# nobkagit/NeuralSteganography

Hardware: AMD Instinct MI355X
Metric: payload bits/sec + cover tokens/sec, GPT-2 arithmetic stego at batch, 1-8 GPUs (higher is better)
Workload: dtype f64; 1 GPU; C3 lockstep steps: gpt2 (random-init weights, fp16 compute, f16 logits, fp16 KV cache, batch-invariant native decode step) + ns_encode_step (temp 0.9, precision 26, topk 300), 4096 streams/GPU from a 32-token context, 262 timed lockstep steps (captured hipGraph replays) after 5 untimed, in 1 pass(es) of at most 1024 steps; global_batch=4096, vocab=50257, precision=26, topk=300, parallelism=dp1 (independent streams, no collective), model=gpt2 (random-init), lm_dtype=fp16, logits_dtype=f16, payload_bytes=1024

## Files before the change

### neuralsteganography_amd/csrc/nsg_coder.hip

```cpp

#include <hip/hip_runtime.h>
#include <stdint.h>
#include <stdio.h>
#include <stdlib.h>
#include <string.h>

#include <algorithm>
#include <string>

#include "../../include/nsg_coder.h"

#pragma clang fp contract(off)

#include "nsg_common.h"
#include "nsg_host.h"
#include "nsg_host.h"

#ifndef NSG_SAMPLE
#define NSG_SAMPLE 64
#endif
#ifndef NSG_FMA_ARG
#define NSG_FMA_ARG 1
#endif
#ifndef NSG_ASM_APPEND
// ... 1443 lines not shown
        s.bit_pos = 0;
        s.ntokens = 0;
        s.flags = 0;
        st[b] = s;
    }
}

}


static thread_local std::string g_err;

static int fail(ns_ctx* ctx, int code, const std::string& msg) {
    if (ctx)
        ctx->err = msg;
    else
        g_err = msg;
    return code;
}

static int g_split_max_b = -2;

static int split_setting() {
    if (g_split_max_b == -2) {
        const char* e = getenv("NSG_SPLIT_MAX_B");
        g_split_max_b = e ? std::max(0, atoi(e)) : -1;
    }
    return g_split_max_b;
}

static int split_max_b(int nsplit) {
    const int v = split_setting();
    return v >= 0 ? v : 6144 / nsplit;
}

template <typename T, bool DECODE, int NSK>
static void launch_one(const nsg::StepParams& p, hipStream_t s) {
    constexpr int NSPLIT = (64 * NSG_SAMPLE) / (nsg::WAVE * nsg::Elem<T>::W);
    if (p.spec_j > 0 && p.B <= split_max_b(NSPLIT)) {
        if (!DECODE && p.stats)
            hipLaunchKernelGGL((nsg::coder_step_kernel<T, DECODE, NSK, !DECODE, NSPLIT>), dim3(p.B),
                               dim3(NSPLIT * nsg::WAVE), 0, s, p);
        else
            hipLaunchKernelGGL((nsg::coder_step_kernel<T, DECODE, NSK, false, NSPLIT>), dim3(p.B),
                               dim3(NSPLIT * nsg::WAVE), 0, s, p);
        return;
    }
    const dim3 grid((p.B + nsg::WPB - 1) / nsg::WPB), block(nsg::WPB * nsg::WAVE);
    if (!DECODE && p.stats)
        hipLaunchKernelGGL((nsg::coder_step_kernel<T, DECODE, NSK, !DECODE>), grid, block, 0, s, p);
    else
        hipLaunchKernelGGL((nsg::coder_step_kernel<T, DECODE, NSK, false>), grid, block, 0, s, p);
}

template <typename T, bool DECODE>
static void launch_t(const nsg::StepParams& p, hipStream_t s) {
    if (p.K <= 128)
        launch_one<T, DECODE, 2>(p, s);
    else if (p.K <= 320)
        launch_one<T, DECODE, 5>(p, s);
    else if (p.K <= 512)
        launch_one<T, DECODE, 8>(p, s);
    else
        launch_one<T, DECODE, (nsg::CAND - nsg::WAVE * 4) / nsg::WAVE>(p, s);
}

template <bool DECODE>
static bool launch(ns_ctx* ctx, const nsg::StepParams& p, hipStream_t s) {
    if (ctx->dtype == NS_DTYPE_F16) {
        if (p.K <= 128)
            launch_one<_Float16, DECODE, 2>(p, s);
        else if (p.K <= 320)
            launch_one<_Float16, DECODE, 5>(p, s);
        else
            launch_one<_Float16, DECODE, (nsg::CAND - nsg::WAVE * 8) / nsg::WAVE>(p, s);
    } else {
        launch_t<float, DECODE>(p, s);
    }
    return hipGetLastError() == hipSuccess;
}

extern "C" {

const char* ns_version(void) { return "nsgcoder 0.25 gfx950"; }

int ns_set_split_max_batch(int max_batch) {
    const int prev = split_setting();
    g_split_max_b = max_batch < 0 ? -1 : max_batch;
    return prev;
}

int ns_max_topk(int logits_dtype) {
    if (logits_dtype == NS_DTYPE_F64) return 0;
    const int TS = (logits_dtype == NS_DTYPE_F16) ? nsg::WAVE * 8 : nsg::WAVE * 4;
    return nsg::CAND - TS;
}

const char* ns_last_error(const ns_ctx* ctx) { return ctx ? ctx->err.c_str() : g_err.c_str(); }

ns_ctx* ns_create(int device, int max_batch, int vocab, int max_k, int precision, int logits_dtype) {
    if (max_batch < 1 || vocab < 2 || max_k < 1 || precision < 1 || precision > 60 ||
        (logits_dtype != NS_DTYPE_F32 && logits_dtype != NS_DTYPE_F16 && logits_dtype != NS_DTYPE_F64)) {
        fail(nullptr, NS_ERR_CONFIG, "ns_create: invalid argument");
        return nullptr;
    }
    if (max_k > ns_max_topk(logits_dtype) && vocab > 0x1FFFF) {
        fail(nullptr, NS_ERR_UNSUPPORTED, "ns_create: the wide (large top-k) path supports vocab < 131072");
        return nullptr;
    }
    if (hipSetDevice(device) != hipSuccess) {
        fail(nullptr, NS_ERR_HIP, "ns_create: hipSetDevice failed");
        return nullptr;
    }
    ns_ctx* ctx = new ns_ctx();
    ctx->device = device;
    ctx->max_batch = max_batch;
    ctx->vocab = vocab;
    ctx->max_k = max_k;
    ctx->precision = precision;
    ctx->dtype = logits_dtype;
    ctx->d_counters = nullptr;
    ctx->wide = NsgWide();
    ctx->sent_end = nullptr;
    ctx->stats = nullptr;
    ctx->ranked = nullptr;
    ctx->ranked_stride = 0;
    ctx->stamps = nullptr;
    ctx->rk_count = nullptr;
    ctx->rk_idmap = nullptr;
    ctx->rk_idmap_stride = 0;
    ctx->rk_dict = 0;
    const size_t cbytes = 4 * NS_COUNTER_SHARDS * sizeof(unsigned long long);
    if (hipMalloc((void**)&ctx->d_counters, cbytes) != hipSuccess || hipMemset(ctx->d_counters, 0, cbytes) != hipSuccess) {
        fail(nullptr, NS_ERR_HIP, "ns_create: hipMalloc failed");
        delete ctx;
        return nullptr;
    }
    if (max_k > ns_max_topk(logits_dtype) && nsg_wide_alloc(ctx) != NS_OK) {
        fail(nullptr, NS_ERR_HIP, "ns_create: allocation of the wide-path scratch failed");
        nsg_wide_free(ctx);
        (void)hipFree(ctx->d_counters);
        delete ctx;
        return nullptr;
    }
    return ctx;
}

void ns_destroy(ns_ctx* ctx) {
    if (!ctx) return;
    if (ctx->d_counters) (void)hipFree(ctx->d_counters);
    nsg_wide_free(ctx);
    delete ctx;
}

int ns_init_state(ns_ctx* ctx, ns_stream_state* d_state, int B, void* hip_stream) {
    if (!ctx || !d_state || B < 1 || B > ctx->max_batch) return fail(ctx, NS_ERR_CONFIG, "ns_init_state: bad argument");
    const int threads = 256;
    hipLaunchKernelGGL(nsg::init_state_kernel, dim3((B + threads - 1) / threads), dim3(threads), 0,
                       (hipStream_t)hip_stream, d_state, B, ctx->precision);
    if (hipGetLastError() != hipSuccess) return fail(ctx, NS_ERR_HIP, "ns_init_state: launch failed");
    return NS_OK;
}

static int prepare(ns_ctx* ctx, nsg::StepParams& p, const void* d_logits, int64_t ld, int B, double temp,
                   int topk, const int32_t* banned, int nbanned, ns_step_trace* d_trace, uint32_t flags,
                   ns_stream_state* d_state) {
    if (!ctx) return fail(ctx, NS_ERR_CONFIG, "null context");
// ... 290 lines not shown
```

### neuralsteganography_amd/csrc/nsg_lm.hip

```cpp

#include <hip/hip_runtime.h>
#include <stdint.h>

#include "nsg_coder.h"
#include "nsg_lm.h"

namespace nsg {
namespace lm {

typedef _Float16 f16;
typedef _Float16 f16x8 __attribute__((ext_vector_type(8)));
typedef _Float16 f16x4 __attribute__((ext_vector_type(4)));
typedef float f32x4 __attribute__((ext_vector_type(4)));

constexpr int BK = 64;

__device__ __forceinline__ f32x4 mfma16(f16x8 a, f16x8 b, f32x4 c) {
    return __builtin_amdgcn_mfma_f32_16x16x32_f16(a, b, c, 0, 0, 0);
}

__device__ __forceinline__ float gelu_tanh(float x) {
    const float u = 0.7978845608028654f * (x + 0.044715f * (x * x * x));
    const float e = __builtin_amdgcn_exp2f(u * -2.8853900817779268f);
    return x * __builtin_amdgcn_rcpf(1.0f + e);
}

__device__ __forceinline__ f16 to_f16(float v) {
    asm volatile("" : "+v"(v));
    return (f16)v;
}

template <int EPI>
__device__ __forceinline__ void store4(void* Y, int64_t ldy, const f16* __restrict__ bias, int m, int n, f32x4 acc) {
    float v[4];
    if (bias) {
        const f16x4 bb = *(const f16x4*)(bias + n);
#pragma unroll
        for (int r = 0; r < 4; ++r) v[r] = acc[r] + (float)bb[r];
    } else {
#pragma unroll
        for (int r = 0; r < 4; ++r) v[r] = acc[r];
    }
    if constexpr (EPI == NS_LM_EPI_STORE_F32) {
        float* y = (float*)Y + (int64_t)m * ldy + n;
        *(f32x4*)y = f32x4{v[0], v[1], v[2], v[3]};
    } else {
        f16* y = (f16*)Y + (int64_t)m * ldy + n;
        f16x4 o;
        if constexpr (EPI == NS_LM_EPI_RESIDUAL) {
            const f16x4 h = *(const f16x4*)y;
#pragma unroll
            for (int r = 0; r < 4; ++r) o[r] = to_f16((float)h[r] + v[r]);
        } else if constexpr (EPI == NS_LM_EPI_GELU) {
#pragma unroll
            for (int r = 0; r < 4; ++r) o[r] = to_f16(gelu_tanh(v[r]));
        } else {
#pragma unroll
            for (int r = 0; r < 4; ++r) o[r] = to_f16(v[r]);
        }
        *(f16x4*)y = o;
    }
}

template <int EPI>
__device__ __forceinline__ void store4_pre(void* Y, int64_t ldy, bool has_bias, f16x4 bb, f16x4 h, int m, int n,
                                           f32x4 acc) {
    float v[4];
#pragma unroll
    for (int r = 0; r < 4; ++r) v[r] = has_bias ? acc[r] + (float)bb[r] : acc[r];
    if constexpr (EPI == NS_LM_EPI_STORE_F32) {
        float* y = (float*)Y + (int64_t)m * ldy + n;
        *(f32x4*)y = f32x4{v[0], v[1], v[2], v[3]};
    } else {
        f16* y = (f16*)Y + (int64_t)m * ldy + n;
        f16x4 o;
        if constexpr (EPI == NS_LM_EPI_RESIDUAL) {
#pragma unroll
            for (int r = 0; r < 4; ++r) o[r] = to_f16((float)h[r] + v[r]);
        } else if constexpr (EPI == NS_LM_EPI_GELU) {
#pragma unroll
            for (int r = 0; r < 4; ++r) o[r] = to_f16(gelu_tanh(v[r]));
        } else {
#pragma unroll
            for (int r = 0; r < 4; ++r) o[r] = to_f16(v[r]);
        }
        *(f16x4*)y = o;
    }
}

__host__ __device__ constexpr int k_chains(int K) { return K <= 1024 ? 1 : K <= 2048 ? 2 : 4; }

template <int FM, int SK, int EPI, int NW = 4>
__global__ __launch_bounds__(64 * NW) void gemm_direct(const f16* __restrict__ X, int64_t ldx,
                                                       const f16* __restrict__ Wt, int64_t ldw,
                                                       const f16* __restrict__ bias, void* Y, int64_t ldy, int M, int N,
                                                       int K) {
    static_assert(NW % SK == 0, "a workgroup holds whole weight blocks");
    __shared__ f32x4 s_part[SK > 1 ? NW : 1][SK > 1 ? FM : 1][64];
    const int lane = threadIdx.x & 63, wave = threadIdx.x >> 6;
    const int nb = blockIdx.x * (NW / SK) + wave / SK;
    const int chain = wave % SK;
    const bool live = nb * 16 < N;
    const int m0 = blockIdx.y * 16 * FM;
    const int r = lane & 15, c = lane >> 4;
    const int KT = K / 64, TPC = (KT + SK - 1) / SK;
    const int k_begin = min(chain * TPC, KT) * 64, k_end = min((chain + 1) * TPC, KT) * 64;
    const f16* wrow = Wt + (int64_t)min(nb * 16 + r, N - 1) * ldw + c * 8;
    const f16* xrow[FM];
#pragma unroll
    for (int f = 0; f < FM; ++f) xrow[f] = X + (int64_t)min(m0 + f * 16 + r, M - 1) * ldx + c * 8;
    f32x4 acc[FM];
#pragma unroll
    for (int f = 0; f < FM; ++f) acc[f] = f32x4{0.f, 0.f, 0.f, 0.f};
    const int n = nb * 16 + 4 * c;
    const bool ep = live && n < N && (SK == 1 || chain == 0);
    f16x4 pb = {}, ph[FM];
#pragma unroll
    for (int f = 0; f < FM; ++f) ph[f] = f16x4{};
    if (ep) {
        if (bias) pb = *(const f16x4*)(bias + n);
        if constexpr (EPI == NS_LM_EPI_RESIDUAL) {
#pragma unroll
            for (int f = 0; f < FM; ++f) {
                const int m = m0 + f * 16 + r;
                if (m < M) ph[f] = *(const f16x4*)((const f16*)Y + (int64_t)m * ldy + n);
            }
        }
    }
    constexpr int U = FM == 1 ? 24 : FM == 2 ? 12 : 8;
    int k = k_begin;
    if (live) {
        for (; k + 32 * U <= k_end; k += 32 * U) {
            f16x8 a[U], b[U][FM];
#pragma unroll
            for (int u = 0; u < U; ++u) {
                a[u] = *(const f16x8*)(wrow + k + 32 * u);
#pragma unroll
                for (int f = 0; f < FM; ++f) b[u][f] = *(const f16x8*)(xrow[f] + k + 32 * u);
            }
            __builtin_amdgcn_sched_barrier(0);
#pragma unroll
            for (int u = 0; u < U; ++u)
#pragma unroll
                for (int f = 0; f < FM; ++f) acc[f] = mfma16(a[u], b[u][f], acc[f]);
        }
        for (; k < k_end; k += 32) {
            const f16x8 a = *(const f16x8*)(wrow + k);
#pragma unroll
            for (int f = 0; f < FM; ++f) acc[f] = mfma16(a, *(const f16x8*)(xrow[f] + k), acc[f]);
        }
    }
    if constexpr (SK > 1) {
#pragma unroll
        for (int f = 0; f < FM; ++f) s_part[wave][f][lane] = acc[f];
        __syncthreads();
        if (chain != 0) return;
        for (int q = 1; q < SK; ++q)
#pragma unroll
            for (int f = 0; f < FM; ++f) acc[f] += s_part[wave + q][f][lane];
    }
    if (!ep) return;
#pragma unroll
    for (int f = 0; f < FM; ++f) {
        const int m = m0 + f * 16 + r;
        if (m < M) store4_pre<EPI>(Y, ldy, bias != nullptr, pb, ph[f], m, n, acc[f]);
    }
}

__device__ __forceinline__ int swz(int row) { return (row >> 1) & 7; }
// ... 67 lines not shown
#pragma unroll
    for (int i = 0; i < FN; ++i)
#pragma unroll
        for (int j = 0; j < FM; ++j) acc[i][j] = f32x4{0.f, 0.f, 0.f, 0.f};

    const int KT = K / BK;
    const int SK = k_chains(K), TPC = (KT + SK - 1) / SK;
    const int fr = lane & 15, fc = lane >> 4;
#pragma unroll
    for (int s0 = 0; s0 < NST - 1; ++s0)
        if (s0 < KT) stage(s0, s0);
    int buf = 0;
    for (int kt = 0; kt < KT; ++kt) {
        const int ahead = KT - 1 - kt;
        if constexpr (NST >= 3) {
            if (ahead >= NST - 2) {
                wait_vm<GL * (NST - 2)>();
            } else if (NST >= 4 && ahead == 1) {
                wait_vm<GL>();
            } else {
                wait_vm<0>();
            }
            __builtin_amdgcn_s_barrier();
            asm volatile("" ::: "memory");
            if (ahead >= NST - 1) {
                int nb = buf + NST - 1;
                nb -= nb >= NST ? NST : 0;
                stage(kt + NST - 1, nb);
            }
        } else {
            if (ahead >= 1) {
                stage(kt + 1, buf ^ 1);
                wait_vm<GL>();
            } else {
                wait_vm<0>();
            }
            __builtin_amdgcn_s_barrier();
            asm volatile("" ::: "memory");
        }
        if constexpr (SPLIT) {
            if (kt > 0 && kt % TPC == 0) {
#pragma unroll
                for (int i = 0; i < FN; ++i)
#pragma unroll
                    for (int j = 0; j < FM; ++j) {
                        tot[i][j] = kt == TPC ? acc[i][j] : tot[i][j] + acc[i][j];
                        acc[i][j] = f32x4{0.f, 0.f, 0.f, 0.f};
                    }
            }
        }
        const char* base = smem + buf * ROWS * 128;
        f16x8 a[2][FN], b[2][FM];
#pragma unroll
        for (int kk = 0; kk < 2; ++kk) {
            const int ch = kk * 4 + fc;
#pragma unroll
            for (int i = 0; i < FN; ++i) {
                const int row = wn * FN * 16 + i * 16 + fr;
                a[kk][i] = *(const f16x8*)(base + row * 128 + ((ch ^ swz(row)) << 4));
            }
#pragma unroll
            for (int j = 0; j < FM; ++j) {
                const int row = BN + wm * FM * 16 + j * 16 + fr;
                b[kk][j] = *(const f16x8*)(base + row * 128 + ((ch ^ swz(row)) << 4));
            }
        }
#pragma unroll
        for (int kk = 0; kk < 2; ++kk)
#pragma unroll
            for (int i = 0; i < FN; ++i)
#pragma unroll
                for (int j = 0; j < FM; ++j) acc[i][j] = mfma16(a[kk][i], b[kk][j], acc[i][j]);
        if constexpr (NST == 2) lds_fence_barrier();
        buf = buf + 1 == NST ? 0 : buf + 1;
    }
    if constexpr (SPLIT) {
        if (KT > TPC) {
#pragma unroll
            for (int i = 0; i < FN; ++i)
#pragma unroll
                for (int j = 0; j < FM; ++j) acc[i][j] = tot[i][j] + acc[i][j];
        }
    }
#pragma unroll
    for (int i = 0; i < FN; ++i) {
        const int n = n0 + wn * FN * 16 + i * 16 + 4 * fc;
        if (n >= N) continue;
#pragma unroll
        for (int j = 0; j < FM; ++j) {
            const int m = m0 + wm * FM * 16 + j * 16 + fr;
            if (m < M) store4<EPI>(Y, ldy, bias, m, n, acc[i][j]);
        }
    }
}

constexpr int PB_BIAS_MAX = 4096;

template <int N_>
__device__ __forceinline__ void wait_vm_le(int n) {
    if constexpr (N_ > 0) {
        if (n >= N_) {
            wait_vm<N_>();
            return;
        }
        wait_vm_le<N_ - 8>(n);
    } else {
        wait_vm<0>();
    }
}

template <int NST, bool SPLIT, int EPI>
__global__ __launch_bounds__(256) void gemm_persist(const f16* __restrict__ X, int64_t ldx,
                                                    const f16* __restrict__ Wt, int64_t ldw,
                                                    const f16* __restrict__ bias, void* Y, int64_t ldy, int M, int N,
                                                    int K) {
    constexpr int BN = 128, BM = 128, WM = 2, NT = 256, NW = 4, FN = 4, FM = 4;
    constexpr int ROWS = BN + BM, GL = ROWS * 8 / NT, SB = ROWS * 128;
    constexpr int NSTO = FN * FM;
    constexpr int ESZ = EPI == NS_LM_EPI_STORE_F32 ? 4 : 2;
    static_assert(NST >= 2 && NST <= 4 && GL == 8, "ring");
    __shared__ __attribute__((aligned(16))) char smem[NST * SB + PB_BIAS_MAX * 2];
    f16* s_bias = (f16*)(smem + NST * SB);

    const int lane = threadIdx.x & 63, wave = threadIdx.x >> 6;
    const int wn = wave / WM, wm = wave - wn * WM;
    const int fr = lane & 15, fc = lane >> 4;
    const int tiles_m = (M + BM - 1) / BM, tiles_n = N / BN, T = tiles_m * tiles_n;
    const int G = gridDim.x, g = xcd_remap(blockIdx.x, G);
    const int KT = K / BK, SK = k_chains(K), TPC = (KT + SK - 1) / SK;
    const int ntl = g < T ? (T - 1 - g) / G + 1 : 0;
    const int S = ntl * KT;

    if (bias) {
        for (int i = threadIdx.x * 8; i < N; i += NT * 8) *(f16x8*)(s_bias + i) = *(const f16x8*)(bias + i);
    }
    __syncthreads();

    auto origin = [&](int i, int& n0, int& m0) {
        constexpr int GN = 1024 / BN;
        const int t = g + i * G;
        const int grp = t / (GN * tiles_m), within = t - grp * (GN * tiles_m);
        const int gn = min(GN, tiles_n - grp * GN);
        const int tm = within / gn;
        n0 = (grp * GN + (within - tm * gn)) * BN;
        m0 = tm * BM;
    };
    const int srow = lane >> 3;
    auto stage = [&](int i, int kt, int buf) {
        int n0, m0;
        origin(i, n0, m0);
        char* dst = smem + buf * SB;
#pragma unroll
        for (int q = 0; q < GL; ++q) {
            const int qq = q * NW + wave;
            const int row = qq * 8 + srow;
            const int chunk = (lane & 7) ^ swz(row);
            const f16* src = q < GL / 2 ? Wt + (int64_t)(n0 + row) * ldw
                                        : X + (int64_t)min(m0 + row - BN, M - 1) * ldx;
            __builtin_amdgcn_global_load_lds((const __attribute__((address_space(1))) void*)(src + chunk * 8 + kt * BK),
                                             (__attribute__((address_space(3))) void*)(dst + qq * 8 * 128), 16, 0, 0);
        }
    };

    const auto rs = __builtin_amdgcn_make_buffer_rsrc(Y, (short)0, (int)((int64_t)M * ldy * ESZ), 0x00020000);

    f32x4 acc[FN][FM];
    f32x4 tot[SPLIT ? FN : 1][SPLIT ? FM : 1];
#pragma unroll
    for (int i = 0; i < FN; ++i)
#pragma unroll
        for (int j = 0; j < FM; ++j) acc[i][j] = f32x4{0.f, 0.f, 0.f, 0.f};

    int is_i = 0, is_k = 0, is_n = 0;
    auto issue = [&]() {
        stage(is_i, is_k, is_n % NST);
        ++is_n;
// ... 230 lines not shown
        char* dst = smem + buf * SB;
        int r8 = wn * 8 + lr;
        asm volatile("" : "+v"(r8));
        if (g == 0) {
#pragma unroll
            for (int q = 0; q < WP + 4; ++q) {
                const f16* p = q < WP ? Wt + (int64_t)min(n0 + q * 32 + r8, N - 1) * ldw
                                      : X + (int64_t)min(m0 + (q - WP) * 32 + r8, M - 1) * ldx;
                __builtin_amdgcn_global_load_lds((const __attribute__((address_space(1))) void*)(p + chunk * 8 + kt * BK),
                                                 (__attribute__((address_space(3))) void*)(dst + (q * 4 + wn) * 1024),
                                                 16, 0, 0);
            }
        } else {
#pragma unroll
            for (int q = 0; q < 4; ++q) {
                const f16* p = X + (int64_t)min(m0 + 128 + q * 32 + r8, M - 1) * ldx;
                __builtin_amdgcn_global_load_lds((const __attribute__((address_space(1))) void*)(p + chunk * 8 + kt * BK),
                                                 (__attribute__((address_space(3))) void*)(dst + ((BN + 128) / 8 + q * 4 + wn) * 1024),
                                                 16, 0, 0);
            }
        }
    };
    auto barrier = []() {
        __builtin_amdgcn_sched_barrier(0);
        __builtin_amdgcn_s_barrier();
        asm volatile("" ::: "memory");
        __builtin_amdgcn_sched_barrier(0);
    };

    f32x4 acc[FN][FM];
#pragma unroll
    for (int i = 0; i < FN; ++i)
#pragma unroll
        for (int j = 0; j < FM; ++j) acc[i][j] = f32x4{0.f, 0.f, 0.f, 0.f};

    const int KT = K / BK;
    stage(0, 0);
    wait_vm<0>();
    barrier();
    if (g == 1) barrier();
    for (int kt = 0; kt < KT; ++kt) {
        const int buf = kt & 1;
        const char* base = smem + buf * SB;
        f16x8 a[2][FN], b[2][FM];
#pragma unroll
        for (int kk = 0; kk < 2; ++kk) {
            const int ch = kk * 4 + fc;
#pragma unroll
            for (int i = 0; i < FN; ++i) {
                const int row = wn * FN * 16 + i * 16 + fr;
                a[kk][i] = *(const f16x8*)(base + row * 128 + ((ch ^ swz(row)) << 4));
            }
#pragma unroll
            for (int j = 0; j < FM; ++j) {
                const int row = BN + g * FM * 16 + j * 16 + fr;
                b[kk][j] = *(const f16x8*)(base + row * 128 + ((ch ^ swz(row)) << 4));
            }
        }
        if (kt + 1 < KT) stage(kt + 1, buf ^ 1);
        asm volatile("s_waitcnt lgkmcnt(0)" ::: "memory");
        barrier();
        __builtin_amdgcn_s_setprio(1);
#pragma unroll
        for (int kk = 0; kk < 2; ++kk)
#pragma unroll
            for (int i = 0; i < FN; ++i)
#pragma unroll
                for (int j = 0; j < FM; ++j) acc[i][j] = mfma16(a[kk][i], b[kk][j], acc[i][j]);
        __builtin_amdgcn_s_setprio(0);
        if (kt + 1 < KT) wait_vm<0>();
        barrier();
    }
    if (g == 0) barrier();
#pragma unroll
    for (int i = 0; i < FN; ++i) {
        const int n = n0 + wn * FN * 16 + i * 16 + 4 * fc;
        if (n >= N) continue;
#pragma unroll
        for (int j = 0; j < FM; ++j) {
            const int m = m0 + g * FM * 16 + j * 16 + fr;
            if (m < M) store4<EPI>(Y, ldy, bias, m, n, acc[i][j]);
        }
    }
}

template <int SK, int EPI>
__global__ __launch_bounds__(256 * SK) void gemm_chains(const f16* __restrict__ X, int64_t ldx,
                                                         const f16* __restrict__ Wt, int64_t ldw,
                                                         const f16* __restrict__ bias, void* Y, int64_t ldy, int M,
                                                         int N, int K) {
    constexpr int BN = 64, BM = 64, WM = 2, FN = 2, FM = 2;
    constexpr int ROWS = BN + BM, GL = ROWS * 8 / 256;
    constexpr int SB = ROWS * 128;
    static_assert(SK == 2 || SK == 4, "chains");
    __shared__ __attribute__((aligned(16))) char smem[SK * 2 * SB];

    const int tiles_m = (M + BM - 1) / BM;
    const int tiles_n = (N + BN - 1) / BN;
    const int t = xcd_remap(blockIdx.x, tiles_m * tiles_n);
    constexpr int GN = 1024 / BN;
    const int grp = t / (GN * tiles_m), within = t - grp * (GN * tiles_m);
    const int gn = min(GN, tiles_n - grp * GN);
    const int tm = within / gn, tn = grp * GN + (within - tm * gn);
    const int n0 = tn * BN, m0 = tm * BM;
    const int lane = threadIdx.x & 63;
    const int wave = __builtin_amdgcn_readfirstlane(threadIdx.x >> 6);
    const int c = wave >> 2, ww = wave & 3;
    const int wn = ww / WM, wm = ww - wn * WM;
    char* ring = smem + c * 2 * SB;

    const f16* src[GL];
    int lds_off[GL];
#pragma unroll
    for (int g = 0; g < GL; ++g) {
        const int q = g * 4 + ww;
        const int row = q * 8 + (lane >> 3);
        const int chunk = (lane & 7) ^ swz(row);
        if (row < BN)
            src[g] = Wt + (int64_t)min(n0 + row, N - 1) * ldw + chunk * 8;
        else
            src[g] = X + (int64_t)min(m0 + row - BN, M - 1) * ldx + chunk * 8;
        lds_off[g] = q * 8 * 128;
    }
    auto stage = [&](int kt, int buf) {
#pragma unroll
        for (int g = 0; g < GL; ++g)
            __builtin_amdgcn_global_load_lds((const __attribute__((address_space(1))) void*)(src[g] + kt * BK),
                                             (__attribute__((address_space(3))) void*)(ring + buf * SB + lds_off[g]),
                                             16, 0, 0);
    };

    f32x4 acc[FN][FM];
#pragma unroll
    for (int i = 0; i < FN; ++i)
#pragma unroll
        for (int j = 0; j < FM; ++j) acc[i][j] = f32x4{0.f, 0.f, 0.f, 0.f};
    const int KT = K / BK, TPC = (KT + SK - 1) / SK;
    const int k0 = c * TPC, nk = max(0, min(k0 + TPC, KT) - k0);
    const int fr = lane & 15, fc = lane >> 4;
    if (nk > 0) stage(k0, 0);
    int buf = 0;
    for (int i = 0; i < TPC; ++i) {
        if (i + 1 < nk) {
            stage(k0 + i + 1, buf ^ 1);
            wait_vm<GL>();
        } else {
            wait_vm<0>();
        }
        __builtin_amdgcn_s_barrier();
        asm volatile("" ::: "memory");
        if (i < nk) {
            const char* base = ring + buf * SB;
            f16x8 a[2][FN], b[2][FM];
#pragma unroll
            for (int kk = 0; kk < 2; ++kk) {
                const int ch = kk * 4 + fc;
#pragma unroll
                for (int ii = 0; ii < FN; ++ii) {
                    const int row = wn * FN * 16 + ii * 16 + fr;
                    a[kk][ii] = *(const f16x8*)(base + row * 128 + ((ch ^ swz(row)) << 4));
                }
#pragma unroll
                for (int j = 0; j < FM; ++j) {
                    const int row = BN + wm * FM * 16 + j * 16 + fr;
                    b[kk][j] = *(const f16x8*)(base + row * 128 + ((ch ^ swz(row)) << 4));
                }
// ... 152 lines not shown
            for (int e = 0; e < 4; ++e) {
                h[e] = ok ? (f16)((float)te[e] + (float)tp[e]) : (f16)__builtin_nanf("");
                x[v][e] = (float)h[e];
            }
            *(f16x4*)(hr + 4 * i) = h;
        }
    }
    ln_row(x, NV4, C, w, b, A + (int64_t)row * lda, eps);
}


constexpr int LNG_MAXK = 1024;
template <int EPI, int NW = 4>
__global__ __launch_bounds__(64 * NW) void gemm_direct_ln(const f16* __restrict__ X, int64_t ldx,
                                                          const f16* __restrict__ lw, const f16* __restrict__ lb,
                                                          float eps, const f16* __restrict__ Wt, int64_t ldw,
                                                          const f16* __restrict__ bias, void* Y, int64_t ldy, int M,
                                                          int N, int K) {
    __shared__ __attribute__((aligned(16))) f16 sA[16][LNG_MAXK + 8];
    const int lane = threadIdx.x & 63, wave = threadIdx.x >> 6;
    const int nb = blockIdx.x * NW + wave;
    const bool live = nb * 16 < N;
    const int r = lane & 15, c = lane >> 4;
    const int KS = K / 32;
    const f16* wrow = Wt + (int64_t)min(nb * 16 + r, N - 1) * ldw + c * 8;
    f16x8 a[LNG_MAXK / 32];
    if (live) {
#pragma unroll
        for (int u = 0; u < LNG_MAXK / 32; ++u)
            if (u < KS) a[u] = *(const f16x8*)(wrow + 32 * u);
    }
    const int n = nb * 16 + 4 * c;
    const bool ep = live && n < N;
    f16x4 pb = {}, ph = {};
    if (ep) {
        if (bias) pb = *(const f16x4*)(bias + n);
        if constexpr (EPI == NS_LM_EPI_RESIDUAL) {
            if (r < M) ph = *(const f16x4*)((const f16*)Y + (int64_t)r * ldy + n);
        }
    }
    const int NV4 = K >> 2;
    for (int row = wave; row < M; row += NW) {
        const f16* xr = X + (int64_t)row * ldx;
        float x[LN_MAXV][4];
#pragma unroll
        for (int v = 0; v < LN_MAXV; ++v) {
            const int i = lane + 64 * v;
            if (i < NV4) {
                const f16x4 t = *(const f16x4*)(xr + 4 * i);
#pragma unroll
                for (int e = 0; e < 4; ++e) x[v][e] = (float)t[e];
            }
        }
        ln_row(x, NV4, K, lw, lb, &sA[row][0], eps);
    }
    __syncthreads();
    if (!ep) return;
    const f16* arow = &sA[min(r, M - 1)][c * 8];
    f32x4 acc = f32x4{0.f, 0.f, 0.f, 0.f};
#pragma unroll
    for (int u = 0; u < LNG_MAXK / 32; ++u)
        if (u < KS) acc = mfma16(a[u], *(const f16x8*)(arow + 32 * u), acc);
    if (r < M) store4_pre<EPI>(Y, ldy, bias != nullptr, pb, ph, r, n, acc);
}

}
}

using namespace nsg::lm;

enum GemmCfg {
    CFG_DIRECT16 = 0, CFG_DIRECT32, CFG_DIRECT64,
    CFG_T64_2, CFG_T64_3,
    CFG_T128_2, CFG_T128_3, CFG_T128_4,
    CFG_T256x128_2, CFG_T256x128_3,
    CFG_T128x256_2,
    CFG_T64_4,
    CFG_T128x64_3,
    CFG_B256,
    CFG_P128_2, CFG_P128_3, CFG_P128_4,
    CFG_PP256,
    CFG_PP192,
    CFG_C64,
    CFG_COUNT
};

static int cu_count() {
    static int n = 0;
    if (n == 0) {
        int dev = 0, v = 0;
        if (hipGetDevice(&dev) == hipSuccess &&
            hipDeviceGetAttribute(&v, hipDeviceAttributeMultiprocessorCount, dev) == hipSuccess && v > 0)
            n = v;
        else
            n = 256;
    }
    return n;
}

static bool persist_ok(int epi, const void* bias, int64_t ldy, int M, int N) {
    const int64_t esz = epi == NS_LM_EPI_STORE_F32 ? 4 : 2;
    return epi != NS_LM_EPI_RESIDUAL && N % 128 == 0 && (!bias || N <= PB_BIAS_MAX) &&
           ((int64_t)M + 128) * ldy * esz < ((int64_t)1 << 31);
}

#ifndef NSG_DIRECT_NW
#define NSG_DIRECT_NW 1
#endif

template <int FM, int EPI>
static void launch_direct(const f16* x, int64_t ldx, const f16* wt, int64_t ldw, const f16* bias, void* y,
                          int64_t ldy, int M, int N, int K, hipStream_t st) {
    const int nbk = N / 16, my = (M + 16 * FM - 1) / (16 * FM);
    constexpr int NW1 = NSG_DIRECT_NW;
    switch (k_chains(K)) {
        case 1:
            hipLaunchKernelGGL((gemm_direct<FM, 1, EPI, NW1>), dim3((nbk + NW1 - 1) / NW1, my), dim3(64 * NW1), 0, st,
                               x, ldx, wt, ldw, bias, y, ldy, M, N, K);
            break;
        case 2:
            hipLaunchKernelGGL((gemm_direct<FM, 2, EPI>), dim3((nbk + 1) / 2, my), dim3(256), 0, st, x, ldx, wt, ldw,
                               bias, y, ldy, M, N, K);
            break;
        default:
            hipLaunchKernelGGL((gemm_direct<FM, 4, EPI>), dim3(nbk, my), dim3(256), 0, st, x, ldx, wt, ldw, bias, y,
                               ldy, M, N, K);
            break;
    }
}

template <int EPI>
static void launch_cfg(int cfg, const f16* x, int64_t ldx, const f16* wt, int64_t ldw, const f16* bias, void* y,
                       int64_t ldy, int M, int N, int K, hipStream_t st) {
    auto tiles = [&](int bn, int bm) { return dim3((unsigned)(((M + bm - 1) / bm) * (long)((N + bn - 1) / bn))); };
    const bool split = k_chains(K) > 1;
    switch (cfg) {
#define NSG_DIRECT(FMv) launch_direct<FMv, EPI>(x, ldx, wt, ldw, bias, y, ldy, M, N, K, st)
#define NSG_TILED(BNv, BMv, WNv, WMv, NSTv)                                                                     \
    if (split)                                                                                                  \
        hipLaunchKernelGGL((gemm_tiled<BNv, BMv, WNv, WMv, NSTv, true, EPI>), tiles(BNv, BMv), dim3(64 * WNv * WMv), \
                           0, st, x, ldx, wt, ldw, bias, y, ldy, M, N, K);                                      \
    else                                                                                                        \
        hipLaunchKernelGGL((gemm_tiled<BNv, BMv, WNv, WMv, NSTv, false, EPI>), tiles(BNv, BMv),                 \
                           dim3(64 * WNv * WMv), 0, st, x, ldx, wt, ldw, bias, y, ldy, M, N, K)
        case CFG_DIRECT16: NSG_DIRECT(1); break;
        case CFG_DIRECT32: NSG_DIRECT(2); break;
        case CFG_DIRECT64: NSG_DIRECT(4); break;
        case CFG_T64_2: NSG_TILED(64, 64, 2, 2, 2); break;
        case CFG_T64_3: NSG_TILED(64, 64, 2, 2, 3); break;
        case CFG_T128_2: NSG_TILED(128, 128, 2, 2, 2); break;
        case CFG_T128_3: NSG_TILED(128, 128, 2, 2, 3); break;
        case CFG_T128_4: NSG_TILED(128, 128, 2, 2, 4); break;
        case CFG_T256x128_2: NSG_TILED(256, 128, 4, 2, 2); break;
        case CFG_T256x128_3: NSG_TILED(256, 128, 4, 2, 3); break;
        case CFG_T128x256_2: NSG_TILED(128, 256, 2, 4, 2); break;
        case CFG_T64_4: NSG_TILED(64, 64, 2, 2, 4); break;
        case CFG_T128x64_3: NSG_TILED(128, 64, 2, 2, 3); break;
        case CFG_B256:
            if (split) {
                NSG_TILED(128, 128, 2, 2, 2);
            } else {
                hipLaunchKernelGGL((gemm_big<EPI>), tiles(256, 256), dim3(512), 0, st, x, ldx, wt, ldw, bias, y, ldy,
                                   M, N, K);
            }
            break;
        case CFG_PP256:
            if (split) {
                NSG_TILED(128, 128, 2, 2, 2);
            } else {
                hipLaunchKernelGGL((gemm_pp<EPI>), tiles(256, 256), dim3(512), 0, st, x, ldx, wt, ldw, bias, y, ldy, M,
                                   N, K);
            }
            break;
        case CFG_PP192:
            if (split) {
                NSG_TILED(128, 128, 2, 2, 2);
            } else {
                hipLaunchKernelGGL((gemm_pp<EPI, 192>), tiles(192, 256), dim3(512), 0, st, x, ldx, wt, ldw, bias, y,
                                   ldy, M, N, K);
            }
            break;
        case CFG_C64: {
            const int sk = k_chains(K);
            if (sk == 4)
                hipLaunchKernelGGL((gemm_chains<4, EPI>), tiles(64, 64), dim3(1024), 0, st, x, ldx, wt, ldw, bias, y, ldy,
                                   M, N, K);
            else if (sk == 2)
                hipLaunchKernelGGL((gemm_chains<2, EPI>), tiles(64, 64), dim3(512), 0, st, x, ldx, wt, ldw, bias, y, ldy,
                                   M, N, K);
            else
                NSG_TILED(64, 64, 2, 2, 2);
            break;
        }
        case CFG_P128_2:
        case CFG_P128_3:
        case CFG_P128_4: {
            if (!persist_ok(EPI, bias, ldy, M, N)) {
                NSG_TILED(128, 128, 2, 2, 2);
                break;
            }
            const int T = ((M + 127) / 128) * (N / 128);
            const int G = min(T, cu_count() * (cfg == CFG_P128_2 ? 2 : 1));
            if constexpr (EPI != NS_LM_EPI_RESIDUAL) {
#define NSG_PERSIST(NSTv)                                                                                        \
    if (split)                                                                                                   \
        hipLaunchKernelGGL((gemm_persist<NSTv, true, EPI>), dim3(G), dim3(256), 0, st, x, ldx, wt, ldw, bias, y, \
                           ldy, M, N, K);                                                                        \
    else                                                                                                         \
        hipLaunchKernelGGL((gemm_persist<NSTv, false, EPI>), dim3(G), dim3(256), 0, st, x, ldx, wt, ldw, bias, y, \
                           ldy, M, N, K)
                if (cfg == CFG_P128_2) {
                    NSG_PERSIST(2);
                } else if (cfg == CFG_P128_3) {
                    NSG_PERSIST(3);
                } else {
                    NSG_PERSIST(4);
                }
#undef NSG_PERSIST
            }
            break;
        }
#undef NSG_DIRECT
#undef NSG_TILED
        default: break;
    }
}

static int auto_cfg(int M, int N, int K) {
    const bool split = k_chains(K) > 1;
    if (M <= 16) return (N >= 8192 && !split) ? CFG_T64_2 : CFG_DIRECT16;
    if (split && M <= 256) return M <= 64 ? CFG_DIRECT16 : M <= 128 ? CFG_DIRECT32 : CFG_DIRECT64;
    if (N >= 8192 && M >= 512) return (!split && M < 2048) ? CFG_PP256 : CFG_T128_2;
    if (!split && M >= 4096 && N >= 2048) {
        const long cu = cu_count(), tm = (M + 255) / 256;
        const long w256 = (tm * ((N + 255) / 256) + cu - 1) / cu * 256;
        const long w192 = (tm * ((N + 191) / 192) + cu - 1) / cu * 192;
        return w192 < w256 ? CFG_PP192 : CFG_PP256;
    }
    if (!split && M >= 1024 && N >= 4096) return CFG_T128x64_3;
    if (split && (long)((M + 63) / 64) * ((N + 63) / 64) <= 2L * cu_count()) return CFG_C64;
    return CFG_T64_2;
}

static int gemm_checked(const void* d_x, int64_t ldx, const void* d_wt, int64_t ldw, const void* d_bias, void* d_y,
                        int64_t ldy, int M, int N, int K, int epilogue, int cfg, void* hip_stream) {
    if (!d_x || !d_wt || !d_y || M <= 0 || N <= 0 || K <= 0) return NS_ERR_CONFIG;
    if (K % 64 || N % 16) return NS_ERR_UNSUPPORTED;
    if (ldx < K || ldw < K || ldy < N) return NS_ERR_CONFIG;
    const uintptr_t al = (uintptr_t)d_x | (uintptr_t)d_wt | (uintptr_t)d_y | (uintptr_t)(d_bias ? d_bias : d_x);
    if ((al & 15u) || (ldx & 7) || (ldw & 7) || (ldy & 3)) return NS_ERR_CONFIG;
    if ((int64_t)((M + 15) / 16) * ((N + 15) / 16) > 0x7FFFFFFF) return NS_ERR_UNSUPPORTED;
    if (cfg < 0) cfg = auto_cfg(M, N, K);
    if (cfg >= CFG_COUNT) return NS_ERR_CONFIG;
    const f16 *x = (const f16*)d_x, *wt = (const f16*)d_wt, *b = (const f16*)d_bias;
    const hipStream_t st = (hipStream_t)hip_stream;
    switch (epilogue) {
        case NS_LM_EPI_STORE: launch_cfg<NS_LM_EPI_STORE>(cfg, x, ldx, wt, ldw, b, d_y, ldy, M, N, K, st); break;
        case NS_LM_EPI_GELU: launch_cfg<NS_LM_EPI_GELU>(cfg, x, ldx, wt, ldw, b, d_y, ldy, M, N, K, st); break;
        case NS_LM_EPI_RESIDUAL: launch_cfg<NS_LM_EPI_RESIDUAL>(cfg, x, ldx, wt, ldw, b, d_y, ldy, M, N, K, st); break;
        case NS_LM_EPI_STORE_F32: launch_cfg<NS_LM_EPI_STORE_F32>(cfg, x, ldx, wt, ldw, b, d_y, ldy, M, N, K, st); break;
        default: return NS_ERR_CONFIG;
    }
    return hipGetLastError() == hipSuccess ? NS_OK : NS_ERR_HIP;
}

extern "C" int ns_lm_gemm(const void* d_x, int64_t ldx, const void* d_wt, int64_t ldw, const void* d_bias, void* d_y,
                          int64_t ldy, int M, int N, int K, int epilogue, void* hip_stream) {
    return gemm_checked(d_x, ldx, d_wt, ldw, d_bias, d_y, ldy, M, N, K, epilogue, -1, hip_stream);
}

extern "C" int ns_lm_gemm_config(const void* d_x, int64_t ldx, const void* d_wt, int64_t ldw, const void* d_bias,
                                 void* d_y, int64_t ldy, int M, int N, int K, int epilogue, int config,
                                 void* hip_stream) {
    return gemm_checked(d_x, ldx, d_wt, ldw, d_bias, d_y, ldy, M, N, K, epilogue, config, hip_stream);
}

extern "C" int ns_lm_gemm_configs(void) { return CFG_COUNT; }

extern "C" int ns_lm_layernorm_count(const void* d_x, int64_t ldx, const void* d_w, const void* d_b, void* d_y,
                                     int64_t ldy, int M, int C, float eps, int32_t* d_counter, void* hip_stream) {
    if (!d_x || !d_w || !d_b || !d_y || M <= 0 || C <= 0) return NS_ERR_CONFIG;
    if (C % 4 || C > 256 * LN_MAXV) return NS_ERR_UNSUPPORTED;
    const uintptr_t al = (uintptr_t)d_x | (uintptr_t)d_w | (uintptr_t)d_b | (uintptr_t)d_y;
    if ((al & 7u) || (ldx & 3) || (ldy & 3) || ldx < C || ldy < C || ((uintptr_t)d_counter & 3u)) return NS_ERR_CONFIG;
    hipLaunchKernelGGL(layernorm_kernel, dim3((M + 3) / 4), dim3(256), 0, (hipStream_t)hip_stream, (const f16*)d_x,
                       ldx, (const f16*)d_w, (const f16*)d_b, (f16*)d_y, ldy, M, C, eps, d_counter, nullptr);
    return hipGetLastError() == hipSuccess ? NS_OK : NS_ERR_HIP;
}

extern "C" int ns_lm_layernorm(const void* d_x, int64_t ldx, const void* d_w, const void* d_b, void* d_y, int64_t ldy,
                               int M, int C, float eps, void* hip_stream) {
    return ns_lm_layernorm_count(d_x, ldx, d_w, d_b, d_y, ldy, M, C, eps, nullptr, hip_stream);
}

extern "C" int ns_lm_ln_gemm(const void* d_x, int64_t ldx, const void* d_lw, const void* d_lb, float eps,
                             const void* d_wt, int64_t ldw, const void* d_bias, void* d_y, int64_t ldy, int M, int N,
                             int K, int epilogue, void* d_a, int64_t lda, void* hip_stream) {
    if (!d_x || !d_lw || !d_lb || !d_wt || !d_y || M <= 0 || N <= 0 || K <= 0) return NS_ERR_CONFIG;
    const bool fused = M <= 16 && K <= LNG_MAXK && K % 64 == 0 && N % 16 == 0 && auto_cfg(M, N, K) == CFG_DIRECT16;
    if (!fused) {
        if (!d_a) return NS_ERR_CONFIG;
        const int rc = ns_lm_layernorm(d_x, ldx, d_lw, d_lb, d_a, lda, M, K, eps, hip_stream);
        if (rc != NS_OK) return rc;
        return gemm_checked(d_a, lda, d_wt, ldw, d_bias, d_y, ldy, M, N, K, epilogue, -1, hip_stream);
    }
    if (ldx < K || ldw < K || ldy < N) return NS_ERR_CONFIG;
    const uintptr_t al = (uintptr_t)d_x | (uintptr_t)d_wt | (uintptr_t)d_y | (uintptr_t)(d_bias ? d_bias : d_x) |
                         (uintptr_t)d_lw | (uintptr_t)d_lb;
    if ((al & 15u) || (ldx & 7) || (ldw & 7) || (ldy & 3)) return NS_ERR_CONFIG;
    const f16 *x = (const f16*)d_x, *wt = (const f16*)d_wt, *b = (const f16*)d_bias, *lw = (const f16*)d_lw,
              *lb = (const f16*)d_lb;
    const hipStream_t st = (hipStream_t)hip_stream;
    constexpr int NW1 = NSG_DIRECT_NW;
    const dim3 grid((N / 16 + NW1 - 1) / NW1), blk(64 * NW1);
    switch (epilogue) {
        case NS_LM_EPI_STORE:
            hipLaunchKernelGGL((gemm_direct_ln<NS_LM_EPI_STORE, NW1>), grid, blk, 0, st, x, ldx, lw, lb, eps, wt, ldw, b,
                               d_y, ldy, M, N, K);
            break;
        case NS_LM_EPI_GELU:
// ... 75 lines not shown
```

Measured before the change: 5.957 million payload bits/s.

## Add phased-prefetch 256x256 GEMM kernel and route large GEMMs to it

Adds gemm_ph, a 256xBN tile GEMM that splits each K-step into four phases. Each phase issues part of the next tiles' global-to-LDS loads, with fine-grained vmcnt waits between MFMA groups, so memory traffic interleaves with compute instead of arriving in bulk. It also adds a store_frags epilogue that preloads bias and residual fragments before storing. The auto config switches M>=4096, N>=2048 non-split GEMMs from PP kernels to PH kernels. The risks are higher register pressure from the FN x 8 accumulators and more barriers per K-step.

```diff
diff --git a/neuralsteganography_amd/csrc/nsg_coder.hip b/neuralsteganography_amd/csrc/nsg_coder.hip
--- a/neuralsteganography_amd/csrc/nsg_coder.hip
+++ b/neuralsteganography_amd/csrc/nsg_coder.hip
@@ -1549,7 +1549,7 @@
 
 extern "C" {
 
-const char* ns_version(void) { return "nsgcoder 0.25 gfx950"; }
+const char* ns_version(void) { return "nsgcoder 0.26 gfx950"; }
 
 int ns_set_split_max_batch(int max_batch) {
     const int prev = split_setting();
diff --git a/neuralsteganography_amd/csrc/nsg_lm.hip b/neuralsteganography_amd/csrc/nsg_lm.hip
--- a/neuralsteganography_amd/csrc/nsg_lm.hip
+++ b/neuralsteganography_amd/csrc/nsg_lm.hip
@@ -85,6 +85,38 @@
             for (int r = 0; r < 4; ++r) o[r] = to_f16(v[r]);
         }
         *(f16x4*)y = o;
+    }
+}
+
+template <int EPI, int FN, int FM>
+__device__ __forceinline__ void store_frags(void* Y, int64_t ldy, const f16* __restrict__ bias, int M, int N, int nb,
+                                            int mb, int fr, int fc, const f32x4 (&acc)[FN][FM]) {
+    f16x4 bb[FN], h[EPI == NS_LM_EPI_RESIDUAL ? FN : 1][EPI == NS_LM_EPI_RESIDUAL ? FM : 1];
+#pragma unroll
+    for (int i = 0; i < FN; ++i) {
+        const int n = nb + i * 16 + 4 * fc;
+        bb[i] = f16x4{};
+        if (bias && n < N) bb[i] = *(const f16x4*)(bias + n);
+        if constexpr (EPI == NS_LM_EPI_RESIDUAL) {
+#pragma unroll
+            for (int j = 0; j < FM; ++j) {
+                const int m = mb + j * 16 + fr;
+                h[i][j] = f16x4{};
+                if (n < N && m < M) h[i][j] = *(const f16x4*)((const f16*)Y + (int64_t)m * ldy + n);
+            }
+        }
+    }
+#pragma unroll
+    for (int i = 0; i < FN; ++i) {
+        const int n = nb + i * 16 + 4 * fc;
+        if (n >= N) continue;
+#pragma unroll
+        for (int j = 0; j < FM; ++j) {
+            const int m = mb + j * 16 + fr;
+            f16x4 hv = f16x4{};
+            if constexpr (EPI == NS_LM_EPI_RESIDUAL) hv = h[i][j];
+            if (m < M) store4_pre<EPI>(Y, ldy, bias != nullptr, bb[i], hv, m, n, acc[i][j]);
+        }
     }
 }
 
@@ -318,16 +350,7 @@
                 for (int j = 0; j < FM; ++j) acc[i][j] = tot[i][j] + acc[i][j];
         }
     }
-#pragma unroll
-    for (int i = 0; i < FN; ++i) {
-        const int n = n0 + wn * FN * 16 + i * 16 + 4 * fc;
-        if (n >= N) continue;
-#pragma unroll
-        for (int j = 0; j < FM; ++j) {
-            const int m = m0 + wm * FM * 16 + j * 16 + fr;
-            if (m < M) store4<EPI>(Y, ldy, bias, m, n, acc[i][j]);
-        }
-    }
+    store_frags<EPI>(Y, ldy, bias, M, N, n0 + wn * FN * 16, m0 + wm * FM * 16, fr, fc, acc);
 }
 
 constexpr int PB_BIAS_MAX = 4096;
@@ -724,6 +747,143 @@
             if (m < M) store4<EPI>(Y, ldy, bias, m, n, acc[i][j]);
         }
     }
+}
+
+template <int EPI, int BN = 256>
+__global__ __launch_bounds__(512) void gemm_ph(const f16* __restrict__ X, int64_t ldx, const f16* __restrict__ Wt,
+                                               int64_t ldw, const f16* __restrict__ bias, void* Y, int64_t ldy, int M,
+                                               int N, int K) {
+    static_assert(BN == 256 || BN == 192, "weight panel");
+    constexpr int BM = 256, FN = BN / 64, FM = 8, SB = (BN + BM) * 128;
+    constexpr int WP = BN / 64;
+    constexpr int SZ0 = 2, SZ1 = WP - 2, SZ2 = 2, SZ3 = 2;
+    constexpr int NA = SZ3 + SZ0 + SZ1, NB = SZ0 + SZ1 + SZ2 + SZ3;
+    __shared__ __attribute__((aligned(16))) char smem[2 * SB];
+
+    const int tiles_m = (M + BM - 1) / BM, tiles_n = (N + BN - 1) / BN;
+    const int t = xcd_remap(blockIdx.x, tiles_m * tiles_n);
+    constexpr int GN = 4;
+    const int grp = t / (GN * tiles_m), within = t - grp * (GN * tiles_m);
+    const int gn = min(GN, tiles_n - grp * GN);
+    const int tm = within / gn, tn = grp * GN + (within - tm * gn);
+    const int n0 = tn * BN, m0 = tm * BM;
+    const int lane = threadIdx.x & 63;
+    const int wave = __builtin_amdgcn_readfirstlane(threadIdx.x >> 6);
+    const int g = wave >> 2, wn = wave & 3;
+    const int fr = lane & 15, fc = lane >> 4;
+    const int lr = lane >> 3;
+    const int chunk = (lane & 7) ^ ((wn * 4 + (lane >> 4)) & 7);
+    const f16* pw[WP];
+    const f16* px[4];
+#pragma unroll
+    for (int q = 0; q < WP; ++q) pw[q] = Wt + (int64_t)min(n0 + q * 64 + wave * 8 + lr, N - 1) * ldw + chunk * 8;
+#pragma unroll
+    for (int q = 0; q < 4; ++q)
+        px[q] = X + (int64_t)min(m0 + g * 128 + q * 32 + wn * 8 + lr, M - 1) * ldx + chunk * 8;
+    auto piece_w = [&](int q, int kt, int buf) {
+        __builtin_amdgcn_global_load_lds((const __attribute__((address_space(1))) void*)(pw[q] + kt * BK),
+                                         (__attribute__((address_space(3))) void*)(smem + buf * SB +
+                                                                                   (q * 64 + wave * 8) * 128),
+                                         16, 0, 0);
+    };
+    auto piece_x = [&](int q, int kt, int buf) {
+        __builtin_amdgcn_global_load_lds((const __attribute__((address_space(1))) void*)(px[q] + kt * BK),
+                                         (__attribute__((address_space(3))) void*)(smem + buf * SB +
+                                                                                   (BN + g * 128 + q * 32 + wn * 8) * 128),
+                                         16, 0, 0);
+    };
+    auto unit = [&](int u, int kt, int buf) {
+        if (u == 0) {
+            piece_w(0, kt, buf);
+            piece_w(1, kt, buf);
+        } else if (u == 1) {
+#pragma unroll
+            for (int q = 2; q < WP; ++q) piece_w(q, kt, buf);
+        } else {
+            piece_x(2 * (u - 2), kt, buf);
+            piece_x(2 * (u - 2) + 1, kt, buf);
+        }
+    };
+    auto barrier = []() {
+        __builtin_amdgcn_sched_barrier(0);
+        __builtin_amdgcn_s_barrier();
+        asm volatile("" ::: "memory");
+        __builtin_amdgcn_sched_barrier(0);
+    };
+
+    f32x4 acc[FN][FM];
+#pragma unroll
+    for (int i = 0; i < FN; ++i)
+#pragma unroll
+        for (int j = 0; j < FM; ++j) acc[i][j] = f32x4{0.f, 0.f, 0.f, 0.f};
+
+    const int KT = K / BK;
+#pragma unroll
+    for (int u = 0; u < 4; ++u) unit(u, 0, 0);
+    if (KT > 1) {
+        unit(0, 1, 1);
+        unit(1, 1, 1);
+        wait_vm<NA>();
+    } else {
+        wait_vm<SZ3>();
+    }
+    barrier();
+    if (g == 1) barrier();
+    for (int kt = 0; kt < KT; ++kt) {
+        const int buf = kt & 1;
+        const char* base = smem + buf * SB;
+        f16x8 a[2][FN];
+#pragma unroll
+        for (int p = 0; p < 4; ++p) {
+            f16x8 b[2][2];
+#pragma unroll
+            for (int kk = 0; kk < 2; ++kk) {
+                const int ch = kk * 4 + fc;
+                if (p == 0) {
+#pragma unroll
+                    for (int i = 0; i < FN; ++i) {
+                        const int row = wn * FN * 16 + i * 16 + fr;
+                        a[kk][i] = *(const f16x8*)(base + row * 128 + ((ch ^ swz(row)) << 4));
+                    }
+                }
+#pragma unroll
+                for (int j = 0; j < 2; ++j) {
+                    const int row = BN + g * FM * 16 + (2 * p + j) * 16 + fr;
+                    b[kk][j] = *(const f16x8*)(base + row * 128 + ((ch ^ swz(row)) << 4));
+                }
+            }
+            if (p < 2) {
+                if (kt + 1 < KT) unit(p + 2, kt + 1, buf ^ 1);
+            } else {
+                if (kt + 2 < KT) unit(p - 2, kt + 2, buf);
+            }
+            if (p == 1) {
+                if (kt + 1 < KT)
+                    wait_vm<NB>();
+                else
+                    wait_vm<0>();
+            }
+            if (p == 3) {
+                if (kt + 2 < KT)
+                    wait_vm<NA>();
+                else if (kt + 1 < KT)
+                    wait_vm<SZ3>();
+            }
+            asm volatile("s_waitcnt lgkmcnt(0)" ::: "memory");
+            barrier();
+            __builtin_amdgcn_s_setprio(1);
+#pragma unroll
+            for (int kk = 0; kk < 2; ++kk)
+#pragma unroll
+                for (int i = 0; i < FN; ++i)
+#pragma unroll
+                    for (int j = 0; j < 2; ++j) acc[i][2 * p + j] = mfma16(a[kk][i], b[kk][j], acc[i][2 * p + j]);
+            __builtin_amdgcn_s_setprio(0);
+            barrier();
+        }
+    }
+    if (g == 0) barrier();
+    store_frags<EPI>(Y, ldy, bias, M, N, n0 + wn * FN * 16, m0 + g * FM * 16, fr, fc, acc);
 }
 
 template <int SK, int EPI>
@@ -1042,6 +1202,8 @@
     CFG_PP256,
     CFG_PP192,
     CFG_C64,
+    CFG_T96x128_3, CFG_T96x128_4,
+    CFG_PH256, CFG_PH192,
     CFG_COUNT
 };
 
@@ -1140,6 +1302,24 @@
                                    ldy, M, N, K);
             }
             break;
+        case CFG_T96x128_3: NSG_TILED(96, 128, 2, 2, 3); break;
+        case CFG_T96x128_4: NSG_TILED(96, 128, 2, 2, 4); break;
+        case CFG_PH256:
+            if (split) {
+                NSG_TILED(128, 128, 2, 2, 2);
+            } else {
+                hipLaunchKernelGGL((gemm_ph<EPI>), tiles(256, 256), dim3(512), 0, st, x, ldx, wt, ldw, bias, y, ldy, M,
+                                   N, K);
+            }
+            break;
+        case CFG_PH192:
+            if (split) {
+                NSG_TILED(128, 128, 2, 2, 2);
+            } else {
+                hipLaunchKernelGGL((gemm_ph<EPI, 192>), tiles(192, 256), dim3(512), 0, st, x, ldx, wt, ldw, bias, y,
+                                   ldy, M, N, K);
+            }
+            break;
         case CFG_C64: {
             const int sk = k_chains(K);
             if (sk == 4)
@@ -1195,7 +1375,7 @@
         const long cu = cu_count(), tm = (M + 255) / 256;
         const long w256 = (tm * ((N + 255) / 256) + cu - 1) / cu * 256;
         const long w192 = (tm * ((N + 191) / 192) + cu - 1) / cu * 192;
-        return w192 < w256 ? CFG_PP192 : CFG_PP256;
+        return w192 < w256 ? CFG_PH192 : CFG_PH256;
     }
     if (!split && M >= 1024 && N >= 4096) return CFG_T128x64_3;
     if (split && (long)((M + 63) / 64) * ((N + 63) / 64) <= 2L * cu_count()) return CFG_C64;
```

Result: faster. 6.030 million payload bits/s, median of 6 (+1.2%).
